# medvedevgroup/vargeno

Measured on AMD Instinct MI355X. Metric: reads/sec genotyped (whole node), hg38+dbSNP 30×; achieved HBM GB/s vs peak, higher is better.
Workload: dtype u64

## Files before the change

include/vargeno_hip.h:

```cpp
#ifndef VARGENO_HIP_H
#define VARGENO_HIP_H
#include <stddef.h>
#include <stdint.h>
#ifdef __cplusplus
extern "C" {
#endif

#define VG_OK        0
#define VG_EINVAL   -1
#define VG_EIO      -2
#define VG_ENOMEM   -3
#define VG_ENODEV   -4
#define VG_ETOOBIG  -5
#define VG_EBADREAD -6

typedef struct vg_index vg_index;

typedef struct {
	uint64_t n_ref;            const uint64_t *ref_kmer;  const uint32_t *ref_pos;  const uint8_t *ref_amb;
	uint64_t n_ref_aux;        const uint32_t *ref_aux;
	uint64_t n_snp;            const uint64_t *snp_kmer;  const uint32_t *snp_pos;
	const uint8_t *snp_info;   const uint8_t *snp_amb;    const uint8_t *snp_rf;    const uint8_t *snp_af;
	uint64_t n_snp_aux;        const uint32_t *snp_aux_pos;
	                           const uint8_t  *snp_aux_info;
// ... 122 lines not shown

int  vg_fastq_stream_begin_gzip(vg_index *ix);
int  vg_gzip_stream_stats(vg_index *ix, vg_gzip_stats *stats);
int  vg_fastq_stream_gzip_checkpoint(vg_index *ix, uint64_t text_offset, uint64_t *comp_bit_offset, uint64_t *ckpt_text_offset, uint8_t *window, uint32_t *window_len);

int  vg_fastq_submit(vg_index *ix, const uint8_t *text, uint64_t nbytes,
                     uint64_t *n_records, uint64_t *consumed, uint64_t *last_record_start);

typedef struct vg_packer vg_packer;
int  vg_packer_create(int host_threads, vg_packer **out);
void vg_packer_destroy(vg_packer *pk);
int  vg_packer_begin(vg_packer *pk);
uint64_t vg_packer_reads_cap(uint64_t nbytes);
uint64_t vg_packer_kmers_cap(uint64_t nbytes);
int  vg_packer_push(vg_packer *pk, const uint8_t *text, uint64_t nbytes, uint64_t *kmers, uint64_t kmers_cap, uint64_t *meta,
                    uint64_t *chunk_offsets, uint64_t reads_cap, uint64_t *n_reads, uint64_t *n_chunks, uint64_t *n_invalid);
int  vg_packer_end(vg_packer *pk, uint64_t *n_records, uint64_t *consumed, uint64_t *last_record_start, int *refused);

int  vg_sync(vg_index *ix);
int  vg_stats_get(vg_index *ix, vg_stats *out);
int  vg_set_stats(vg_index *ix, int enable);
int  vg_timing_get(vg_index *ix, vg_timing *out);
uint64_t vg_held_passes(const vg_index *ix);

uint64_t vg_num_sites(const vg_index *ix);
int  vg_sites_fetch(vg_index *ix, uint32_t *pos, uint8_t *ref_base, uint8_t *alt_base,
                    uint8_t *ref_freq, uint8_t *alt_freq);
int  vg_counts_fetch(vg_index *ix, uint8_t *ref_cnt, uint8_t *alt_cnt);
int  vg_counts_reset(vg_index *ix);

int  vg_sample_calls_fetch(vg_index *ix, uint8_t *gt, int32_t *gq, uint64_t *n_escaped);
int  vg_call_device(int device, const uint8_t *ref_cnt, const uint8_t *alt_cnt, const uint8_t *ref_freq, const uint8_t *alt_freq,
                    uint64_t n, double guard, uint8_t *gt, int32_t *gq, uint64_t *n_escaped);

typedef struct vg_gmatrix vg_gmatrix;
int  vg_gmatrix_create(int device, uint64_t n_sites, uint32_t n_samples, vg_gmatrix **out);
int  vg_gmatrix_set(vg_gmatrix *gm, uint32_t sample, const uint8_t *gt, const int32_t *gq, int32_t min_gq);
int  vg_gmatrix_pairs(vg_gmatrix *gm, uint64_t words_per_block, uint64_t *counts);
uint64_t vg_gmatrix_device_bytes(const vg_gmatrix *gm);
void vg_gmatrix_destroy(vg_gmatrix *gm);
int  vg_pairs_host(const uint8_t *gt, const int32_t *gq, uint64_t n_sites, uint32_t n_samples, int32_t min_gq, int threads, uint64_t *counts);

#ifndef VG_CPRIOR_ITERS
#define VG_CPRIOR_ITERS     8
#define VG_CPRIOR_PSEUDO    2.0
#define VG_CPRIOR_ITERS_MAX 64
// ... 80 lines not shown
```

vargeno_amd/_lib.py:

```python
from __future__ import annotations

import ctypes as C
import os

HERE = os.path.dirname(os.path.abspath(__file__))
LIB_PATH = os.environ.get("VARGENO_HIP_LIB") or os.path.join(HERE, "csrc", "libvargeno_hip.so")

VG_ERRORS = {-1: "VG_EINVAL", -2: "VG_EIO", -3: "VG_ENOMEM", -4: "VG_ENODEV", -5: "VG_ETOOBIG", -6: "VG_EBADREAD"}

STAT_FIELDS = ["reads", "reads_n", "reads_invalid", "passes", "passes_ok", "chunks", "gate_open",
               "refbf_pos", "snpbf_pos", "large_block", "ref_query", "snp_query", "ref_probe", "snp_probe",
               "scan_ref", "scan_snp", "scan_oob", "aux_ref", "aux_snp", "site_test", "ctx", "walks", "incr",
               "ingest_bytes", "overflow_reads", "overflow_deep", "alg_bytes"]

SYMBOLS = ["vg_last_error", "vg_build_id", "vg_device_count", "vg_device_memory", "vg_share_budget", "vg_link_rate", "vg_host_alloc_pinned", "vg_host_free_pinned", "vg_index_open", "vg_index_open_ex", "vg_index_plan", "vg_index_open_report", "vg_index_create", "vg_index_close",
           "vg_index_device_bytes", "vg_index_views", "vg_reads_submit", "vg_reads_process_device", "vg_reads_process_device_gated", "vg_reads_submit_packed", "vg_reads_submit_packed_async", "vg_read_store_create", "vg_read_store_push", "vg_read_store_flush", "vg_read_store_reads", "vg_read_store_bytes_used", "vg_reads_submit_store", "vg_read_store_destroy", "vg_fastq_submit", "vg_fastq_stream_begin", "vg_fastq_stream_begin_packed", "vg_fastq_stream_push", "vg_fastq_stream_end",
           "vg_packer_create", "vg_packer_destroy", "vg_packer_begin", "vg_packer_reads_cap", "vg_packer_kmers_cap", "vg_packer_push", "vg_packer_end", "vg_sync", "vg_stats_get",
           "vg_set_stats", "vg_timing_get", "vg_num_sites", "vg_sites_fetch", "vg_counts_fetch", "vg_counts_reset",
           "vg_counts_device_ptr", "vg_counts_allreduce", "vg_counts_allreduce_devices",
           "vg_samples_reserve", "vg_num_samples", "vg_sample_select", "vg_sample_selected", "vg_sample_reset", "vg_sample_invalid_reads",
           "vg_fastq_stream_begin_bgzf", "vg_fastq_stream_bgzf_locate", "vg_bgzf_inflate_device", "vg_bgzf_inflate_host", "vg_bgzf_scan_host",
           "vg_bgzf_deflate_bound", "vg_bgzf_deflate_host", "vg_bgzf_deflate_device",
           "vg_bgzf_deflate_host_coded", "vg_bgzf_deflate_device_coded", "vg_deflate_code_lengths_host", "vg_deflate_code_lengths_device",
           "vg_sample_calls_fetch", "vg_call_device",
           "vg_fastq_stream_begin_bam", "vg_bam_stream_stats", "vg_bam_frame_device", "vg_bam_to_fastq_host",
           "vg_gunzip_host", "vg_gunzip_device", "vg_gunzip_chunked_host", "vg_gunzip_pushed_host",
           "vg_fastq_stream_begin_gzip", "vg_gzip_stream_stats", "vg_fastq_stream_gzip_checkpoint",
           "vg_gmatrix_create", "vg_gmatrix_set", "vg_gmatrix_pairs", "vg_gmatrix_device_bytes", "vg_gmatrix_destroy", "vg_pairs_host",
           "vg_cprior_create", "vg_cprior_set", "vg_cprior_run", "vg_cprior_calls", "vg_cprior_device_bytes", "vg_cprior_destroy", "vg_cprior_host",
           "vg_jtext_create", "vg_jtext_destroy", "vg_jtext_device_bytes", "vg_jtext_set", "vg_jtext_text_bound", "vg_jtext_bgzf_bound", "vg_jtext_render", "vg_jtext_render_host",
           "vg_jtext_bgzf_begin", "vg_jtext_bgzf_text", "vg_jtext_bgzf_lines", "vg_jtext_bgzf_end",
           "vg_vcfidx_create", "vg_vcfidx_destroy", "vg_vcfidx_text_host", "vg_vcfidx_text_device", "vg_vcfidx_bgzf", "vg_vcfidx_bound", "vg_vcfidx_finish", "vg_vcfidx_error", "vg_vcfidx_stats",
           "vg_bgzf_deflate_device_indexed", "vg_jtext_bgzf_index",
           "vg_jtext_create_info", "vg_jtext_text_bound_info", "vg_jtext_render_host_info", "vg_jtext_counts", "vg_jtext_counts_host",
           "vg_held_passes"]

GZIP_STAT_FIELDS = ["members", "chunks", "guessed", "confirmed", "repaired", "tested", "slots_refused", "resume_bit"]


class VgStats(C.Structure):
    _fields_ = [(n, C.c_uint64) for n in STAT_FIELDS]

    def as_dict(self):
        return {n: int(getattr(self, n)) for n in STAT_FIELDS}


class VgGzipStats(C.Structure):
    _fields_ = [(n, C.c_uint64) for n in GZIP_STAT_FIELDS]

    def as_dict(self):
        return {n: int(getattr(self, n)) for n in GZIP_STAT_FIELDS}


class VgGzipOpts(C.Structure):
    _fields_ = [(n, C.c_uint64) for n in ("chunk_bytes", "slot_bytes", "max_ratio", "slot_max")]


class VgTiming(C.Structure):
# ... 183 lines not shown
        L.vg_vcfidx_text_host.argtypes = [vp, vp, C.c_uint64, C.c_int]
        L.vg_vcfidx_text_device.argtypes = [vp, C.c_int, vp, C.c_uint64]
        L.vg_vcfidx_bgzf.argtypes = [vp, vp, C.c_uint64]
        L.vg_vcfidx_bound.argtypes = [vp]
        L.vg_vcfidx_bound.restype = C.c_uint64
        L.vg_vcfidx_finish.argtypes = [vp, vp, C.c_uint64, C.POINTER(C.c_uint64)]
        L.vg_vcfidx_error.argtypes = [vp, C.POINTER(C.c_uint64)]
        L.vg_vcfidx_error.restype = C.c_char_p
        L.vg_vcfidx_stats.argtypes = [vp, vp]
        L.vg_bgzf_deflate_device_indexed.argtypes = [C.c_int, vp, C.c_uint64, C.c_uint32, C.c_int, C.c_int, vp, vp, C.c_uint64, C.POINTER(C.c_uint64)]
        L.vg_jtext_bgzf_index.argtypes = [vp, vp]
        L.vg_jtext_create_info.argtypes = [C.c_int, C.c_uint64, C.c_uint32, C.c_uint32, C.c_uint64, C.c_uint64, C.c_uint64, C.c_int, C.c_int, C.POINTER(vp)]
        L.vg_jtext_text_bound_info.argtypes = [C.c_uint64, C.c_uint64, C.c_uint32, C.c_int]
        L.vg_jtext_text_bound_info.restype = C.c_uint64
        L.vg_jtext_render_host_info.argtypes = [C.c_uint64, C.c_uint32, vp, vp, vp, C.c_uint64, vp, C.c_uint64, vp, C.c_uint64, C.c_int, C.c_int, vp, C.c_uint64, C.POINTER(C.c_uint64), C.POINTER(C.c_uint64)]
        L.vg_jtext_counts.argtypes = [vp, vp, C.c_uint64, vp, C.c_uint64, vp]
        L.vg_jtext_counts_host.argtypes = [C.c_uint64, C.c_uint32, vp, vp, vp, C.c_uint64, vp, C.c_uint64, vp]
        try:
            L.vg_held_passes.argtypes = [vp]
            L.vg_held_passes.restype = C.c_uint64
        except AttributeError:
            if not os.environ.get("VARGENO_HIP_LIB"):
                raise
        if not os.environ.get("VARGENO_HIP_LIB"):
            want = source_build_id()
            got = L.vg_build_id().decode()
            if want is not None and got != want:
                raise RuntimeError("stale %s: built from sources with id %s, the sources next to it have id %s -- rebuild with "
                                   "`python -c 'import __graft_entry__ as g; g.build()'`" % (LIB_PATH, got, want))
        _lib = L
    return _lib


LIB_SOURCES = [os.path.join(HERE, "..", "include", "vargeno_hip.h")] + [os.path.join(HERE, "csrc", f) for f in ("vg_device.h", "vg_wave.h", "vargeno_hip.hip", "vg_sort.hip", "vg_arena.h", "vg_hostpack.h", "vg_hostpack.cpp", "vg_allreduce_plan.h", "vg_hostpack_impl.h", "vg_hostpack_impl.inc", "vg_hostpack_avx2.cpp")]


def source_build_id():
    import hashlib

    h = hashlib.sha256()
    try:
        for f in LIB_SOURCES:
            with open(f, "rb") as fh:
                h.update(fh.read())
    except OSError:
        return None
# ... 7 lines not shown
```

vargeno_amd/api.py:

```python
from __future__ import annotations

import collections
import ctypes as C
import os
import re

import numpy as np

from . import _lib
from ._lib import VgIndexArrays, VgStats, VgTiming, check, lib


def _ptr(a):
    return a.ctypes.data_as(C.c_void_p)


class GenoIndex:

    def __init__(self, handle, device):
        self._h = handle
        self.device = device
        self._stores = []

    @classmethod
# ... 158 lines not shown
        self._stores = []

    def set_stats(self, enable):
        check(lib().vg_set_stats(self._h, 1 if enable else 0))

    def stats(self):
        s = VgStats()
        check(lib().vg_stats_get(self._h, C.byref(s)))
        return s.as_dict()

    def timing(self):
        t = VgTiming()
        check(lib().vg_timing_get(self._h, C.byref(t)))
        return dict(ms_total=float(t.ms_total), ms_pack=float(t.ms_pack), ms_main=float(t.ms_main), ms_tail=float(t.ms_tail), ms_deep_lists=float(t.ms_deep_lists), batches=int(t.batches))

    @property
    def held_passes(self):
        fn = getattr(lib(), "vg_held_passes", None)
        if fn is None:
            raise RuntimeError("the library named by VARGENO_HIP_LIB predates vg_held_passes")
        return int(fn(self._h))

    @property
    def num_sites(self):
        return int(lib().vg_num_sites(self._h))

    @property
    def device_bytes(self):
        return int(lib().vg_index_device_bytes(self._h))

    VIEW_NAMES = {1: "sec", 2: "mx", 4: "dx", 8: "snp_probe", 16: "snp_jg32", 32: "hx", 64: "snp_sig", 128: "sec_is_bf", 256: "ssec"}

    @property
    def views(self):
        m = int(lib().vg_index_views(self._h))
        return [n for b, n in sorted(self.VIEW_NAMES.items()) if m & b]

    def sites(self):
        n = self.num_sites
        pos = np.empty(n, np.uint32)
        u8 = [np.empty(n, np.uint8) for _ in range(4)]
        check(lib().vg_sites_fetch(self._h, _ptr(pos), *[_ptr(x) for x in u8]))
        return dict(pos=pos, ref_base=u8[0], alt_base=u8[1], ref_freq=u8[2], alt_freq=u8[3])

    def reserve_samples(self, n):
        check(lib().vg_samples_reserve(self._h, int(n)))
# ... 744 lines not shown
```

vargeno_amd/csrc/vargeno_hip.hip:

```cpp
#include "../../include/vargeno_hip.h"
#include "vg_device.h"
#include "vg_wave.h"
#include "vg_hostpack.h"
#include "vg_allreduce_plan.h"
#include "vg_arena.h"
#include "vg_inflate.h"
#include "vg_deflate.h"
#include "vg_bam.h"
#include "vg_gunzip.h"
#include "vg_caller.h"
#include "vg_pairs.h"
#include "vg_cprior.h"
#include "vg_jtext.h"
#include "vg_vcfidx.h"

#include <dlfcn.h>
#include <hip/hip_runtime.h>
#include <fcntl.h>
#include <stdio.h>
#include <stdlib.h>
#include <string.h>
#include <sys/stat.h>
#include <unistd.h>

// ... 1596 lines not shown
	LateStore late;
	uint32_t late_h[4] = {0, 0, 0, 0};
	bool late_dirty = false, late_stats = false;
	uint64_t late_reads_run = 0;
	bool spill_known = false;
	uint32_t spill_hint = 0;
	uint64_t cum[4] = {0, 0, 0, 0};
	uint8_t *d_clamped = nullptr;
	void *d_call_block = nullptr;
	const uint8_t *d_site_rf = nullptr, *d_site_af = nullptr;
	uint16_t *d_calls = nullptr;
	const vg_caller_tables *d_call_tab = nullptr;
	unsigned long long *d_call_esc = nullptr;
	unsigned long long *d_stats = nullptr;
	bool stats_enabled = true;
	bool force_generic = false;
	double t_pack = 0, t_main = 0, t_tail = 0, t_total = 0, t_w2 = 0; uint64_t t_batches = 0;
	int cus = 256;
	int lane_grid_blocks = 0, wave_grid = 0;
	uint32_t work_chunk = 128;
	uint32_t hold_pairs = VG_HOLD_PAIRS_DEFAULT;
	uint32_t wave_wgs = 0;
	uint64_t held_passes = 0;
	uint32_t w2_chunk = 8, w2_wpc = 3;
	bool w2_full_grid = false;
	FqStream *d_fq = nullptr;
	bool fq_open = false; int fq_prev_slot = -1;
	BgzfStream bz;
	bool fq_bgzf = false;
	struct GzipStream *gz = nullptr;
	bool fq_gzip = false;
	uint64_t max_device_bytes = 0;
	std::string plan_text;
	std::string aux_note;
	std::string open_report;
	vgp::Packer *packer = nullptr;
	bool fq_packed = false;
	uint64_t host_invalid = 0;
};

static thread_local vg_index *g_building = nullptr;
static thread_local double g_alloc_s = 0;

template <class T>
static int dev_alloc(vg_index *ix, T **p, uint64_t count, bool zero = false, bool plain = false)
{
// ... 1015 lines not shown
	if (!ix) return fail(VG_ENOMEM, "host allocation failed");
	ix->max_device_bytes = max_device_bytes;
	const double t0 = now_s();
	int rc = guarded([&] { return open_impl(prefix, device, ix); });
	if (rc) { vg_index_close(ix); return rc; }
	finish_construction(ix);
	char line[80];
	snprintf(line, sizeof line, "; vg_index_open %.2f s in all", now_s() - t0);
	ix->open_report += line;
	*out = ix;
	return VG_OK;
}

extern "C" const char *vg_index_plan(const vg_index *ix) { return ix ? ix->plan_text.c_str() : ""; }
extern "C" const char *vg_index_open_report(const vg_index *ix) { return ix ? ix->open_report.c_str() : ""; }

extern "C" int vg_index_open(const char *prefix, int device, vg_index **out)
{
	return vg_index_open_ex(prefix, device, env_budget(), out);
}
extern "C" uint64_t vg_index_device_bytes(const vg_index *ix) { return ix ? ix->dev_bytes : 0; }
extern "C" uint64_t vg_num_sites(const vg_index *ix) { return ix ? ix->n_sites : 0; }
extern "C" uint64_t vg_held_passes(const vg_index *ix) { return ix ? ix->held_passes : 0; }
extern "C" uint32_t vg_index_views(const vg_index *ix)
{
	if (!ix) return 0;
	const DevIndex &d = ix->d;
	return (d.sec3 ? VG_VIEW_SEC : 0u) | (d.sec_is_bf ? VG_VIEW_SEC_IS_BF : 0u) | (d.mx ? VG_VIEW_MX : 0u) | (d.dx ? VG_VIEW_DX : 0u) | (d.snp_probe ? VG_VIEW_SNP_PROBE : 0u) | (d.snp_jg32 ? VG_VIEW_SNP_JG32 : 0u) | (d.hx ? VG_VIEW_HX : 0u) | (d.snp_sig ? VG_VIEW_SNP_SIG : 0u) | (d.ssec3 ? VG_VIEW_SSEC : 0u);
}

template <class... A>
static void launch_lane(bool stats, unsigned grid, unsigned block, hipStream_t st, const A &...a)
{
	if (stats) vg_lane_kernel<true><<<grid, block, 0, st>>>(a...);
	else vg_lane_kernel<false><<<grid, block, 0, st>>>(a...);
}

static DevIndex plane_view(const vg_index *ix, uint32_t plane)
{
	DevIndex v = ix->d;
	v.cnt = ix->planes[plane].p.cnt; v.cnt4 = ix->planes[plane].p.cnt4;
	return v;
}

static int harvest(vg_index *ix, Slot &sl)
{
	if (!sl.busy) return VG_OK;
	HIP_TRY(hipEventSynchronize(sl.batch_done));
	const uint32_t resid = sl.lt_late ? sl.h_ctr.p[6] : sl.h_ctr.p[1];
	uint32_t *const r_list = sl.lt_late ? sl.listA.p : sl.listB.p, *const r_cnt = sl.lt_late ? &sl.ctr[6] : &sl.ctr[1];
	if (resid) ix->lane_tier_seen = true;
	if (resid && !sl.lt_enqueued) {
		launch_lane(sl.lt_stats, ix->big.s.nlanes / 64, 64, ix->tail2, plane_view(ix, sl.plane), ix->big.s, sl.lt_bases, sl.lt_quals, sl.lt_offsets, 0, r_list, r_cnt, sl.listC.p, &sl.ctr[2], ix->d_stats, nullptr, sl.lt_gate, sl.pk_kmer.p, sl.pk_meta.p, sl.lt_packed, nullptr, nullptr);
		HIP_TRY(hipGetLastError());
		HIP_TRY(hipMemcpyAsync(sl.h_ctr.p, sl.ctr, 32, hipMemcpyDeviceToHost, ix->tail2));
		HIP_TRY(hipStreamSynchronize(ix->tail2));
	}
	for (int i = 0; i < 4; i++) ix->cum[i] += sl.h_ctr.p[i];
	ix->held_passes += sl.h_ctr.p[CTR_HELD];
	ix->planes[sl.plane].invalid += sl.h_ctr.p[3];
	ix->spill_hint = std::max<uint32_t>(sl.h_ctr.p[0], ix->spill_hint / 2);
	ix->spill_known = true;
	float pack = 0, wave = 0, tail = 0, total = 0, w2 = 0;
	HIP_TRY(hipEventElapsedTime(&pack, sl.pack_begin, sl.pack_end)); HIP_TRY(hipEventElapsedTime(&wave, sl.wave_begin, sl.wave_end));
	HIP_TRY(hipEventElapsedTime(&tail, sl.wave_end, sl.batch_done)); HIP_TRY(hipEventElapsedTime(&total, sl.pack_begin, sl.batch_done)); HIP_TRY(hipEventElapsedTime(&w2, sl.wave_end, sl.deep_end));
	ix->t_pack += pack; ix->t_main += wave; ix->t_tail += tail; ix->t_total += total; ix->t_w2 += w2; ix->t_batches++;
	sl.busy = false;
	return VG_OK;
}

static int run_late_store(vg_index *ix)
{
	if (!ix->late_dirty || !ix->late.state) return VG_OK;
	unsigned long long st[2] = {0, 0};
	HIP_TRY(hipMemcpy(st, ix->late.state, 16, hipMemcpyDeviceToHost));
	ix->late_dirty = false;
	const uint64_t n = st[1];
	if (st[0] == 0) return VG_OK;
	if (n) {
		launch_lane(ix->late_stats, ix->big.s.nlanes / 64, 64, ix->tail, ix->d, ix->big.s, nullptr, nullptr, ix->late.offsets, n, nullptr, nullptr, ix->late.lost, ix->late.lost_n, ix->d_stats, nullptr, nullptr, ix->late.kmers, ix->late.meta, true, ix->d_planes, ix->late.tag);
		HIP_TRY(hipGetLastError());
	}
// ... 101 lines not shown
		if (sl.lt_late) {
			vg_late_collect<<<4, 256, 0, ix->tail>>>(ix->late, sl.pk_kmer.p, sl.pk_meta.p, d_offsets, sl.listB.p, &ctr[1], sl.listA.p, &ctr[6], sl.plane);
			ix->late_dirty = true; ix->late_stats = stats;
		}
	} else {
		sl.lt_late = false;
		const unsigned g1 = (unsigned)std::min<uint64_t>((n_reads + 255) / 256, (uint64_t)ix->lane_grid_blocks);
		if ((rc = begin_batch(sl, ix->stream, produced_on))) return rc;
		HIP_TRY(hipEventRecord(sl.pack_end, ix->stream));
		HIP_TRY(hipEventRecord(sl.wave_begin, ix->stream));
		launch_lane(stats, g1, 256, ix->stream, dv, ix->mid.s, d_bases, d_quals, d_offsets, n_reads, nullptr, d_n_reads, sl.listB.p, &ctr[1], ix->d_stats, packed ? nullptr : &ctr[3], d_gate, sl.pk_kmer.p, sl.pk_meta.p, packed, nullptr, nullptr);
		HIP_TRY(hipEventRecord(sl.wave_end, ix->stream));
		HIP_TRY(hipStreamWaitEvent(ix->tail, sl.wave_end, 0));
	}
	HIP_TRY(hipEventRecord(sl.deep_end, ix->tail));
	sl.lt_bases = d_bases; sl.lt_quals = d_quals; sl.lt_offsets = d_offsets; sl.lt_gate = d_gate; sl.lt_packed = packed; sl.lt_stats = stats;
	sl.lt_enqueued = ix->lane_tier_seen;
	hipStream_t lt = ix->tail;
	if (sl.lt_enqueued) {
		lt = ix->tail2;
		HIP_TRY(hipStreamWaitEvent(lt, sl.deep_end, 0));
		launch_lane(stats, ix->big.s.nlanes / 64, 64, lt, dv, ix->big.s, d_bases, d_quals, d_offsets, 0, sl.lt_late ? sl.listA.p : sl.listB.p, sl.lt_late ? &ctr[6] : &ctr[1], sl.listC.p, &ctr[2], ix->d_stats, nullptr, d_gate, sl.pk_kmer.p, sl.pk_meta.p, packed, nullptr, nullptr);
	}
	HIP_TRY(hipMemcpyAsync(sl.h_ctr.p, ctr, 32, hipMemcpyDeviceToHost, lt));
	HIP_TRY(hipEventRecord(sl.batch_done, lt));
	HIP_TRY(hipGetLastError());
	sl.busy = true;
	return VG_OK;
}

static int acquire_slot(vg_index *ix, Slot **out, uint32_t sample)
{
	Slot &sl = ix->slot[ix->next_slot];
	ix->next_slot = (ix->next_slot + 1) % NSLOT;
	int rc = harvest(ix, sl);
	if (rc) return rc;
	sl.plane = sample;
	*out = &sl;
	return VG_OK;
}

static int size_slot(Slot &sl, uint64_t n_reads, uint64_t n_chunks)
{
	int rc;
	if ((rc = sl.pk_kmer.reserve(n_chunks + 2, "packed reads"))) return rc;
	if ((rc = sl.pk_meta.reserve(n_reads + 1, "packed reads' flag words"))) return rc;
	return reserve_together({&sl.listA, &sl.listB, &sl.listC}, n_reads, "spill lists");
// ... 1669 lines not shown
		HIP_TRY(hipMemset(d_esc.p, 0, sizeof(unsigned long long)));
		vg_call_kernel<<<call_grid(n), VG_CALL_BLOCK>>>(d_cnt.p, d_rf.p, d_af.p, d_tab.p, n, guard, d_code.p, d_esc.p);
		HIP_TRY(hipGetLastError());
		HIP_TRY(hipDeviceSynchronize());
		unsigned long long esc = 0;
		HIP_TRY(hipMemcpy(code.data(), d_code.p, n * sizeof(uint16_t), hipMemcpyDeviceToHost));
		HIP_TRY(hipMemcpy(&esc, d_esc.p, sizeof esc, hipMemcpyDeviceToHost));
		resolve_calls(code.data(), ref_cnt, alt_cnt, ref_freq, alt_freq, n, gt, gq);
		if (n_escaped) *n_escaped = esc;
		return VG_OK;
	});
}

extern "C" int vg_counts_reset(vg_index *ix)
{
	if (!ix) return fail(VG_EINVAL, "null argument");
	{ int rc = finish_pending(ix); if (rc) return rc; }
	HIP_TRY(hipMemsetAsync(ix->d.cnt, 0, (2 * ix->n_sites + 2) * 4, ix->stream));
	for (size_t s = 1; s < ix->planes.size(); s++) HIP_TRY(hipMemsetAsync(ix->planes[s].p.cnt, 0, 2 * ix->n_sites * 4, ix->stream));
	for (Plane &pl : ix->planes) pl.invalid = 0;
	HIP_TRY(hipMemsetAsync(ix->d_stats, 0, S_COUNT * sizeof(unsigned long long), ix->stream));
	for (auto &c : ix->cum) c = 0;
	ix->held_passes = 0;
	ix->host_invalid = 0;
	HIP_TRY(hipStreamSynchronize(ix->stream));
	return VG_OK;
}

extern "C" int vg_counts_device_ptr(vg_index *ix, void **d_counts, uint64_t *n_u32)
{
	if (!ix || !d_counts || !n_u32) return fail(VG_EINVAL, "null argument");
	{ int rc = finish_pending(ix); if (rc) return rc; }
	*d_counts = sel_cnt(ix); *n_u32 = 2 * ix->n_sites;
	return VG_OK;
}

extern "C" uint32_t vg_num_samples(const vg_index *ix) { return ix ? (uint32_t)ix->planes.size() : 0; }
extern "C" uint32_t vg_sample_selected(const vg_index *ix) { return ix ? ix->cur_sample : 0; }
extern "C" int vg_sample_select(vg_index *ix, uint32_t sample)
{
	if (!ix) return fail(VG_EINVAL, "null argument");
	if (sample >= ix->planes.size()) return fail(VG_EINVAL, "sample %s is out of range: the handle has %s plane(s) (vg_samples_reserve)", std::to_string(sample).c_str(), std::to_string(ix->planes.size()).c_str());
	ix->cur_sample = sample;
	return VG_OK;
}
extern "C" int vg_samples_reserve(vg_index *ix, uint32_t n_samples)
// ... 1465 lines not shown
```

vargeno_amd/csrc/vg_wave.h:

```cpp
#pragma once
#include "vg_device.h"
#include "vg_acand.h"

#ifndef VG_WPE
#define VG_WPE 4
#endif
#ifndef VG_SCAN_W
#define VG_SCAN_W 2
#endif

#ifdef VG_STAGE_CLOCKS
#define VG_CLK(i) do { const long long t_ = clock64(); clk[i] += t_ - tlast; tlast = t_; } while (0)
#define VG_CLKW(i) do { __builtin_amdgcn_s_waitcnt(0); VG_CLK(i); } while (0)
#else
#define VG_CLK(i) do { } while (0)
#define VG_CLKW(i) do { } while (0)
#endif

#ifdef VG_STAGE_CLOCKS
__device__ unsigned long long vg_dbg_ovf[8];
#define VG_OVF(r) atomicAdd(&vg_dbg_ovf[(WPB > 1 ? 0 : 4) + (r)], 1ull)
#else
#define VG_OVF(r) do { } while (0)
#endif
// ... 4 lines not shown
#define VG_W1_ECAP 14
#endif
#ifndef VG_W1_NCAP
#define VG_W1_NCAP 6
#endif
#ifndef VG_W1_WPB
#define VG_W1_WPB 4
#endif
constexpr int W1_ECAP = VG_W1_ECAP, W1_NCAP = VG_W1_NCAP, W1_WPB = VG_W1_WPB;
constexpr int W3_ECAP = 48, W3_NCAP = 40;
constexpr uint32_t NOHIT = 0xFFFFFFFFu;
#ifndef VG_SEC_W
#define VG_SEC_W 8
#endif
constexpr int SEC_W = VG_SEC_W;
#ifndef VG_SEC_LONG
#define VG_SEC_LONG 256
#endif
constexpr uint32_t SEC_LONG = VG_SEC_LONG;
constexpr int PCAP = 32;
#ifndef VG_HOLD_PAIRS_DEFAULT
#define VG_HOLD_PAIRS_DEFAULT 12
#endif
constexpr int CTR_WORK_MAIN = 4, CTR_HELD = 7;
constexpr int HCAP = 4;

constexpr uint64_t PK_SKIP_N = 1ull << 62;
constexpr uint64_t PK_INVALID = 1ull << 63;
constexpr uint64_t PK_LONG = 1ull << 61;

__device__ inline uint32_t mk_meta(uint32_t chunk, uint32_t mod, bool neigh, uint32_t nbase) { return chunk | (mod << 5) | ((neigh ? 1u : 0u) << 10) | (nbase << 11); }

struct FuseIn {
	const uint8_t *bases, *quals;
	const uint32_t *gate;
	uint32_t *invalid_reads;
};
#ifndef VG_FUSE_PACK
#define VG_FUSE_PACK 0
#endif

template <bool WIDE> struct XKey { typedef uint32_t type; };
template <> struct XKey<true> { typedef uint64_t type; };
template <bool NARROW> struct KMask { typedef uint32_t type; };
template <> struct KMask<true> { typedef uint16_t type; };

template <bool STATS>
// ... 56 lines not shown
	uint32_t WORK_CHUNK = WORK_CHUNK_ARG;
	if constexpr (WPB == 1) if (read_ids) {
		const uint64_t fair = n_reads / (2ull * gridDim.x * WPB);
		if (fair > WORK_CHUNK) WORK_CHUNK = fair < 16 ? (uint32_t)fair : 16u;
	}
	const uint32_t POOL = WORK_CHUNK * (WPB > 1 ? WPB / 2 : 1);
	const uint32_t work_base = gridDim.x * POOL;
	if (threadIdx.x == 0) {
		const uint64_t p0 = (uint64_t)blockIdx.x * POOL, p1 = p0 + POOL < n_reads ? p0 + POOL : n_reads;
		Q_state = p0 < n_reads ? ((unsigned long long)p1 << 32) | p0 : 0ull;
		Q_lock = 0u; Q_done = 0u;
	}
	__syncthreads();
	uint32_t cursor = 0, end = 0;
	bool drained = false;

	bool active = false;
	constexpr bool HOLD = HOLDK && !STATS && !NOMX && WPB > 1;
	__shared__ uint8_t H_kcnt[HOLD ? 64 * WPB : 1];
	const uint32_t hold_pairs = HOLD ? (HOLD_PAIRS_ARG < (uint32_t)PCAP ? HOLD_PAIRS_ARG : (uint32_t)PCAP) : 0u;
	uint64_t heldm = 0ull;
	uint32_t held_passes = 0;
	const auto held_lane = [&heldm]() -> bool { return HOLD && __builtin_amdgcn_inverse_ballot_w64(heldm); };
#ifdef VG_STAGE_CLOCKS
	long long clk[12] = {0, 0, 0, 0, 0, 0, 0, 0, 0, 0, 0, 0}, tlast = clock64();
	uint32_t iters = 0, dbg_pairs = 0, dbg_items = 0, dbg_rounds = 0, dbg_dq = 0, dbg_rows = 0, dbg_large = 0, dbg_secbad = 0, dbg_holds = 0, dbg_flushes = 0;
#endif
	uint32_t rid = 0, n = 0, gates = 0, pass = 0;
	uint32_t slot0 = 0;
	LaneStats<STATS> tot, cur;
	tot.clear(); cur.clear();

	auto chunk_kmer = [&](uint32_t c) -> uint64_t {
		VG_VC_AS(VC_READS, pk_kmer + ((uint64_t)slot0 + (pass ? n - 1 - c : c)), 8);
		const uint64_t kf = pk_kmer[(uint64_t)slot0 + (pass ? n - 1 - c : c)];
		return pass ? revcomp64(kf) : kf;
	};

	auto chunk_kmer2 = [&](uint32_t c, uint64_t &k0, uint64_t &k1) {
		ulonglong2 v;
		VG_VC_AS(VC_READS, pk_kmer + ((uint64_t)slot0 + (pass ? n - 2 - c : c)), 16);
		__builtin_memcpy(&v, pk_kmer + ((uint64_t)slot0 + (pass ? n - 2 - c : c)), 16);
		k0 = pass ? revcomp64(v.y) : v.x;
		k1 = pass ? revcomp64(v.x) : v.y;
	};

// ... 62 lines not shown
							uint4 t[4];
							#pragma unroll
							for (uint32_t q = 0; q < 4; q++) if (q < 2 || two) t[q] = load_policy<false, uint4, 1>(src + 32 * c0 + 16 * q);
							#pragma unroll
							for (uint32_t z = 0; z < 2; z++) if (z == 0 || two) {
								const uint4 a = t[2 * z], b = t[2 * z + 1];
								const uint64_t k = (uint64_t)pack8(((uint64_t)a.y << 32) | a.x, bad) | ((uint64_t)pack8(((uint64_t)a.w << 32) | a.z, bad) << 16) |
								                   ((uint64_t)pack8(((uint64_t)b.y << 32) | b.x, bad) << 32) | ((uint64_t)pack8(((uint64_t)b.w << 32) | b.z, bad) << 48);
								dst[c0 + z] = k;
							}
						}
						if (fuse.gate) meta = n >= 32 ? fuse.gate[rid] : (fuse.gate[rid] & ((1u << n) - 1u));
						else for (uint32_t c0 = 0; c0 < n && c0 < 32; c0 += 4) {
							uint32_t q4;
							__builtin_memcpy(&q4, fuse.quals + off + c0, 4);
							for (uint32_t j = 0; j < 4 && c0 + j < n && c0 + j < 32; j++) if ((int)(int8_t)(q4 >> (8 * j)) - '8' < 0) meta |= 1ull << (c0 + j);
						}
						if (bad) meta |= classify_bad(src, n) == 1 ? PK_SKIP_N : PK_INVALID;
						if (n > 32) meta |= fuse.gate ? PK_INVALID : PK_LONG;
						if (meta & PK_INVALID) atomicAdd(fuse.invalid_reads, 1u);
						const_cast<uint64_t *>(pk_meta)[rid] = meta;
					} else meta = pk_meta[rid];
					gates = (uint32_t)meta;
					pass = 0;
					cur.clear();
					cur.add(S_READS, 1);
					cur.add(S_INGEST, 9 * n);
					if (meta & (PK_SKIP_N | PK_INVALID)) {
						cur.add((meta & PK_INVALID) ? S_READS_INVALID : S_READS_N, 1);
						if constexpr (STATS) for (int i = 0; i < S_COUNT; i++) tot.v[i] += cur.v[i];
					} else if ((meta & PK_LONG) || n > KMASK_CHUNKS) {
						overflow_list[atomicAdd(overflow_count, 1u)] = rid;
					} else {
						active = true;
					}
				}
			}
			cursor += take;
		}
		if (!__any(active)) { if (drained) break; continue; }
		VG_CLK(0);
#ifdef VG_STAGE_CLOCKS
		iters++;
#endif

		uint32_t kcnt = 0, ncnt = 0;
		uint32_t npend = 0;
		bool ovf = false;
		if (active && !held_lane()) {
			uint32_t hint = 0;
			auto key_find = [&](uint32_t q, uint32_t c, uint32_t lo, uint32_t hi, bool &dup, uint32_t qb = 0u) -> uint32_t {
				uint32_t e = (uint32_t)W_ECAP;
				const uint32_t cnt = hi - lo;
				if (cnt) {
					if (hint < lo || hint >= hi) hint = lo;
					for (uint32_t done = 0; done < cnt && e == (uint32_t)W_ECAP; done += 4) {
						uint32_t v[4], at[4];
						#pragma unroll
						for (uint32_t z = 0; z < 4; z++) { uint32_t i = hint + done + z; if (i >= hi) i -= cnt; if (i >= hi) i = lo; at[z] = i; v[z] = K_idx[i][col]; }
						#pragma unroll
						for (uint32_t z = 0; z < 4; z++) if (e == (uint32_t)W_ECAP && done + z < cnt && v[z] == q) e = at[z];
					}
				}
				if (e != (uint32_t)W_ECAP) {
					const uint32_t m = K_mask[e][col];
					if ((m >> c) & 1u) dup = true; else K_mask[e][col] = (kmask_t)(m | (1u << c) | qb);
					hint = e + 1u;
				}
				return e;
			};
			auto quiet_bit = [&](uint32_t hf, uint32_t c) -> uint32_t { return (hf & 6u) == 0u ? vg_quiet_chunks(hf, c, n) << KFREE : 0u; };
			auto push_exact = [&](uint32_t p, uint32_t c, uint32_t hf = 0u) {
// ... 91 lines not shown
						cur.add(S_CHUNKS, 1);
						emit_exact(c + z, rhit[z] != 0u, rpos[z], rhit[z] >> 1, shit[z] != 0u, spos[z], shit[z] >> 1);
					}
				}
			} else if (use_mx) {
				uint32_t k_strand = 0; bool k_pal = false;
				auto scan_bucket = [&](uint64_t k, uint32_t lo, uint32_t hi, uint4 first, bool &rhit, uint32_t &rpos, uint32_t &ramb, bool &shit, uint32_t &spos, uint32_t &samb) {
					const uint32_t key = (uint32_t)k;
					uint32_t ea = lo;
					if (hi - lo > 4) {
						uint32_t eb = hi;
						while (ea < eb) { const uint32_t m = ea + ((eb - ea) >> 1); if (d.mx[m].x < key) ea = m + 1; else eb = m; }
					}
					for (uint32_t e = ea; e < hi; e++) {
						const uint4 v = (e == lo) ? first : d.mx[e];
						if (v.x < key) continue;
						if (v.x > key) break;
						if (!(k_pal || ((v.z >> 3) & 1u) == k_strand)) continue;
						if (v.z & 1u) { shit = true; spos = v.y; samb = (v.z >> 1) & 1u; }
						else { rhit = true; rpos = v.y; ramb = (v.z >> 1) & 1u; }
					}
				};
				if (d.dx) {
					constexpr uint32_t RC_BAD = 0xFFFFu;
					uint32_t rc_top = pass != 0u ? RC_BAD : (uint32_t)W_ECAP;
					for (uint32_t c = 0; c < n; c += 4) {
						const uint32_t m = n - c < 4u ? n - c : 4u;
						uint64_t kq[4] = {0, 0, 0, 0};
						if (m >= 2) chunk_kmer2(c, kq[0], kq[1]); else kq[0] = chunk_kmer(c);
						if (m >= 4) chunk_kmer2(c + 2, kq[2], kq[3]); else if (m == 3) kq[2] = chunk_kmer(c + 2);
						uint32_t sbits = 0;
						#pragma unroll
						for (uint32_t z = 0; z < 4; z++) {
							const uint64_t kk = kq[z], rr = revcomp64(kk), ck = kk < rr ? kk : rr;
							sbits |= (kk != ck ? 1u : 0u) << z | (kk == rr ? 1u : 0u) << (4u + z);
							kq[z] = fmix64(ck);
						}
						VG_CLKW(9);
						using xkey_t = typename XKey<SDX>::type;
						const uint32_t dxb = SDX ? d.dx_bits : 32u;
						auto ekey = [](const uint4 &e) -> xkey_t { if constexpr (SDX) return ((uint64_t)(e.z & 0xFFFF0000u) << 32) | e.x; else return e.x; };
						auto ecnt = [](const uint4 &b) -> uint32_t { return SDX ? (b.z >> 8) & 0xFFu : b.z >> 8; };
						uint4 bq[4];
						xkey_t kx[4];
						#pragma unroll
						for (uint32_t z = 0; z < 4; z++) {
							bq[z] = make_uint4(0, 0, 0, 0);
// ... 160 lines not shown
										bool dup = false;
										if (key_find(q, cc, rev ? rc_top : 0u, rev ? (uint32_t)W_ECAP : kcnt, dup, qb) == (uint32_t)W_ECAP) {
											if (rev ? rc_top > kcnt : kcnt < (uint32_t)W_ECAP) {
												const uint32_t at = rev ? rc_top - 1u : kcnt;
												K_idx[at][col] = q; K_mask[at][col] = (kmask_t)((1u << cc) | qb);
												if (rev) rc_top = at; else { kcnt++; hint = kcnt; }
											} else if (rev) rc_top = RC_BAD;
											else { VG_OVF(0); ovf = true; }
										} else if (dup) { if (rev) rc_top = RC_BAD; else { VG_OVF(2); ovf = true; } }
									}
								}
							}
							if (!rc_ok) rc_top = RC_BAD;
							if (z0 == 0u) { bq[0] = bq[2]; bq[1] = bq[3]; kx[0] = kx[2]; kx[1] = kx[3]; more[0] = more[2]; more[1] = more[3]; }
						}
#endif
					}
					if (pass == 0u && kcnt == 0u && rc_top != RC_BAD && !ovf) {
						const uint32_t nrc = (uint32_t)W_ECAP - rc_top;
						for (uint32_t i = 0; i < nrc; i++) { K_idx[i][col] = K_idx[rc_top + i][col]; K_mask[i][col] = K_mask[rc_top + i][col]; }
						kcnt = nrc;
						pass = 1u;
					}
				} else
				for (uint32_t c = 0; c < n; c += 2) {
					const bool two = c + 1 < n;
					uint64_t k0 = chunk_kmer(c), k1 = two ? chunk_kmer(c + 1) : 0;
					uint32_t st0, st1; bool pl0, pl1;
					{ const uint64_t r = revcomp64(k0), ck = k0 < r ? k0 : r; st0 = k0 != ck; pl0 = k0 == r; k0 = fmix64(ck); }
					{ const uint64_t r = revcomp64(k1), ck = k1 < r ? k1 : r; st1 = k1 != ck; pl1 = k1 == r; k1 = fmix64(ck); }
					uint32_t lo0, hi0, lo1 = 0, hi1 = 0;
					jg_pair(d.mx_jg, k0 >> 32, lo0, hi0);
					if (two) jg_pair(d.mx_jg, k1 >> 32, lo1, hi1);
					uint4 f0 = make_uint4(0, 0, 0, 0), f1 = f0;
					if (lo0 < hi0) f0 = d.mx[lo0];
					if (lo1 < hi1) f1 = d.mx[lo1];
					uint32_t rpos = 0, ramb = 0, spos = 0, samb = 0;
					bool rhit = false, shit = false;
					cur.add(S_CHUNKS, 1);
					k_strand = st0; k_pal = pl0;
					scan_bucket(k0, lo0, hi0, f0, rhit, rpos, ramb, shit, spos, samb);
					emit_exact(c, rhit, rpos, ramb, shit, spos, samb);
					if (two) {
						rhit = shit = false;
						cur.add(S_CHUNKS, 1);
						k_strand = st1; k_pal = pl1;
// ... 731 lines not shown
							ni++;
							c = mt & 31u; mod = (mt >> 5) & 31u;
							if (wp - 32u * c != target) continue;
						}
						cur.add(S_WALKS, 1);
						if ((uint64_t)wp + 32 > d.pile_len) continue;
						const uint64_t kk = chunk_kmer(c);
						uint4 pw[2];
						load_pile_window(d, wp, pw);
						walk_matches(pw, kk, wp, mod, count);
					}
					}
					}
				}
			}
			if (ovf) {
				overflow_list[atomicAdd(overflow_count, 1u)] = rid;
				active = false;
			} else if (processed || pass == 1) {
				if constexpr (STATS) for (int i = 0; i < S_COUNT; i++) tot.v[i] += cur.v[i];
				active = false;
			} else {
				pass = 1;
			}
		}
		VG_WAVE_SYNC();
		VG_CLK(5);
	}
#ifdef VG_STAGE_CLOCKS
	{ const uint32_t dq = wave_sum<false>(dbg_dq); if (!STATS && lane == 0 && (blockIdx.x % 97u) == 0 && wv == 0) printf("DBG blk %u iters %u pairs %u items %u rounds %u dualq %u large %u secbad %u holds %u flushes %u\n", blockIdx.x, iters, dbg_pairs, dbg_items, dbg_rounds, dq, dbg_large, dbg_secbad, dbg_holds, dbg_flushes); }
	if (!STATS && lane == 0 && (blockIdx.x % 97u) == 0 && wv == 0)
		printf("CLK blk %u iters %u refill %lld A %lld B0 %lld B1 %lld vote %lld walk %lld wload %lld wloop %lld watom %lld Akmer %lld Adx %lld Ascan %lld ecap %d\n", blockIdx.x, iters, clk[0], clk[1], clk[2], clk[3], clk[4], clk[5], clk[6], clk[7], clk[8], clk[9], clk[10], clk[11], W_ECAP);
#endif
	if constexpr (STATS) {
		for (int i = 0; i < S_COUNT; i++) if (tot.v[i]) atomicAdd(&stats[i], (unsigned long long)tot.v[i]);
	}
	if constexpr (HOLD) if (held_passes && lane == 0) atomicAdd(work_next + (CTR_HELD - CTR_WORK_MAIN), held_passes);
}

#undef lane
#undef col

template <bool STATS, int W_ECAP, int W_NCAP, int WPB, bool SDX = false>
__global__ __launch_bounds__(64 * WPB) __attribute__((amdgpu_waves_per_eu(WPB > 1 ? VG_WPE : 1))) void vg_wave_kernel(DevIndex d, const uint64_t *__restrict__ pk_kmer, const uint64_t *__restrict__ pk_meta,
                                                     const uint64_t *__restrict__ offsets, uint64_t n_reads_arg,
                                                     const uint32_t *__restrict__ read_ids, const uint32_t *__restrict__ n_ids,
                                                     uint32_t *overflow_list, uint32_t *overflow_count, uint32_t *work_next, const uint32_t WORK_CHUNK_ARG, const uint32_t HOLD_PAIRS_ARG, unsigned long long *stats, const FuseIn fuse)
{
	vg_wave_body<STATS, W_ECAP, W_NCAP, WPB, false, SDX, true>(d, pk_kmer, pk_meta, offsets, n_reads_arg, read_ids, n_ids, overflow_list, overflow_count, work_next, WORK_CHUNK_ARG, HOLD_PAIRS_ARG, stats, fuse);
}

template <int W_ECAP, int W_NCAP, int WPB, bool SDX>
__global__ __launch_bounds__(64 * WPB) __attribute__((amdgpu_waves_per_eu(WPB > 1 ? VG_WPE : 1))) void vg_wave_kernel_plain(DevIndex d, const uint64_t *__restrict__ pk_kmer, const uint64_t *__restrict__ pk_meta,
                                                     const uint64_t *__restrict__ offsets, uint64_t n_reads_arg,
                                                     const uint32_t *__restrict__ read_ids, const uint32_t *__restrict__ n_ids,
                                                     uint32_t *overflow_list, uint32_t *overflow_count, uint32_t *work_next, const uint32_t WORK_CHUNK_ARG, const uint32_t HOLD_PAIRS_ARG, unsigned long long *stats, const FuseIn fuse)
{
	vg_wave_body<false, W_ECAP, W_NCAP, WPB, false, SDX, false>(d, pk_kmer, pk_meta, offsets, n_reads_arg, read_ids, n_ids, overflow_list, overflow_count, work_next, WORK_CHUNK_ARG, HOLD_PAIRS_ARG, stats, fuse);
}

template <int W_ECAP, int W_NCAP, int WPB>
__global__ __launch_bounds__(64 * WPB) __attribute__((amdgpu_waves_per_eu(WPB > 1 ? VG_WPE : 1))) void vg_wave_kernel_big(DevIndex d, const uint64_t *__restrict__ pk_kmer, const uint64_t *__restrict__ pk_meta,
// ... 9 lines not shown
```

Baseline: 4.006 billion.

## Carry first-pass RC candidate list into retry pass to skip re-lookup

When a read needs a second pass, the kernel now stores the first pass's reverse-complement candidate boundary in the upper 16 bits of the gates word. On retry it compacts the K_idx/K_mask entries and skips the whole lookup stage for that pass. A carried-pass counter is added to the device counters, copied back in a larger counter readback, and exposed through the C and Python APIs. This trades extra register/state bookkeeping and a wider counter copy for avoiding repeated index probing on retried reads.

```diff
diff --git a/include/vargeno_hip.h b/include/vargeno_hip.h
--- a/include/vargeno_hip.h
+++ b/include/vargeno_hip.h
@@ -168,6 +168,7 @@
 int  vg_set_stats(vg_index *ix, int enable);
 int  vg_timing_get(vg_index *ix, vg_timing *out);
 uint64_t vg_held_passes(const vg_index *ix);
+uint64_t vg_carried_passes(const vg_index *ix);
 
 uint64_t vg_num_sites(const vg_index *ix);
 int  vg_sites_fetch(vg_index *ix, uint32_t *pos, uint8_t *ref_base, uint8_t *alt_base,
diff --git a/vargeno_amd/_lib.py b/vargeno_amd/_lib.py
--- a/vargeno_amd/_lib.py
+++ b/vargeno_amd/_lib.py
@@ -33,7 +33,7 @@
            "vg_vcfidx_create", "vg_vcfidx_destroy", "vg_vcfidx_text_host", "vg_vcfidx_text_device", "vg_vcfidx_bgzf", "vg_vcfidx_bound", "vg_vcfidx_finish", "vg_vcfidx_error", "vg_vcfidx_stats",
            "vg_bgzf_deflate_device_indexed", "vg_jtext_bgzf_index",
            "vg_jtext_create_info", "vg_jtext_text_bound_info", "vg_jtext_render_host_info", "vg_jtext_counts", "vg_jtext_counts_host",
-           "vg_held_passes"]
+           "vg_held_passes", "vg_carried_passes"]
 
 GZIP_STAT_FIELDS = ["members", "chunks", "guessed", "confirmed", "repaired", "tested", "slots_refused", "resume_bit"]
 
@@ -263,6 +263,12 @@
         except AttributeError:
             if not os.environ.get("VARGENO_HIP_LIB"):
                 raise
+        try:
+            L.vg_carried_passes.argtypes = [vp]
+            L.vg_carried_passes.restype = C.c_uint64
+        except AttributeError:
+            if not os.environ.get("VARGENO_HIP_LIB"):
+                raise
         if not os.environ.get("VARGENO_HIP_LIB"):
             want = source_build_id()
             got = L.vg_build_id().decode()
diff --git a/vargeno_amd/api.py b/vargeno_amd/api.py
--- a/vargeno_amd/api.py
+++ b/vargeno_amd/api.py
@@ -204,6 +204,13 @@
         return int(fn(self._h))
 
     @property
+    def carried_passes(self):
+        fn = getattr(lib(), "vg_carried_passes", None)
+        if fn is None:
+            raise RuntimeError("the library named by VARGENO_HIP_LIB predates vg_carried_passes")
+        return int(fn(self._h))
+
+    @property
     def num_sites(self):
         return int(lib().vg_num_sites(self._h))
 
diff --git a/vargeno_amd/csrc/vargeno_hip.hip b/vargeno_amd/csrc/vargeno_hip.hip
--- a/vargeno_amd/csrc/vargeno_hip.hip
+++ b/vargeno_amd/csrc/vargeno_hip.hip
@@ -1642,6 +1642,7 @@
 	uint32_t hold_pairs = VG_HOLD_PAIRS_DEFAULT;
 	uint32_t wave_wgs = 0;
 	uint64_t held_passes = 0;
+	uint64_t carried_passes = 0;
 	uint32_t w2_chunk = 8, w2_wpc = 3;
 	bool w2_full_grid = false;
 	FqStream *d_fq = nullptr;
@@ -2703,6 +2704,7 @@
 extern "C" uint64_t vg_index_device_bytes(const vg_index *ix) { return ix ? ix->dev_bytes : 0; }
 extern "C" uint64_t vg_num_sites(const vg_index *ix) { return ix ? ix->n_sites : 0; }
 extern "C" uint64_t vg_held_passes(const vg_index *ix) { return ix ? ix->held_passes : 0; }
+extern "C" uint64_t vg_carried_passes(const vg_index *ix) { return ix ? ix->carried_passes : 0; }
 extern "C" uint32_t vg_index_views(const vg_index *ix)
 {
 	if (!ix) return 0;
@@ -2734,11 +2736,15 @@
 	if (resid && !sl.lt_enqueued) {
 		launch_lane(sl.lt_stats, ix->big.s.nlanes / 64, 64, ix->tail2, plane_view(ix, sl.plane), ix->big.s, sl.lt_bases, sl.lt_quals, sl.lt_offsets, 0, r_list, r_cnt, sl.listC.p, &sl.ctr[2], ix->d_stats, nullptr, sl.lt_gate, sl.pk_kmer.p, sl.pk_meta.p, sl.lt_packed, nullptr, nullptr);
 		HIP_TRY(hipGetLastError());
-		HIP_TRY(hipMemcpyAsync(sl.h_ctr.p, sl.ctr, 32, hipMemcpyDeviceToHost, ix->tail2));
+		HIP_TRY(hipMemcpyAsync(sl.h_ctr.p, sl.ctr, 4 * CTR_COPIED, hipMemcpyDeviceToHost, ix->tail2));
 		HIP_TRY(hipStreamSynchronize(ix->tail2));
 	}
 	for (int i = 0; i < 4; i++) ix->cum[i] += sl.h_ctr.p[i];
 	ix->held_passes += sl.h_ctr.p[CTR_HELD];
+	ix->carried_passes += sl.h_ctr.p[CTR_CARRIED];
+#ifdef VG_RETRY_CENSUS
+	fprintf(stderr, "RETRY_CENSUS carried %u retries %u usable %u usable_empty %u\n", sl.h_ctr.p[CTR_CARRIED], sl.h_ctr.p[CTR_CARRIED + 1], sl.h_ctr.p[CTR_CARRIED + 2], sl.h_ctr.p[CTR_CARRIED + 3]);
+#endif
 	ix->planes[sl.plane].invalid += sl.h_ctr.p[3];
 	ix->spill_hint = std::max<uint32_t>(sl.h_ctr.p[0], ix->spill_hint / 2);
 	ix->spill_known = true;
@@ -2886,7 +2892,7 @@
 		HIP_TRY(hipStreamWaitEvent(lt, sl.deep_end, 0));
 		launch_lane(stats, ix->big.s.nlanes / 64, 64, lt, dv, ix->big.s, d_bases, d_quals, d_offsets, 0, sl.lt_late ? sl.listA.p : sl.listB.p, sl.lt_late ? &ctr[6] : &ctr[1], sl.listC.p, &ctr[2], ix->d_stats, nullptr, d_gate, sl.pk_kmer.p, sl.pk_meta.p, packed, nullptr, nullptr);
 	}
-	HIP_TRY(hipMemcpyAsync(sl.h_ctr.p, ctr, 32, hipMemcpyDeviceToHost, lt));
+	HIP_TRY(hipMemcpyAsync(sl.h_ctr.p, ctr, 4 * CTR_COPIED, hipMemcpyDeviceToHost, lt));
 	HIP_TRY(hipEventRecord(sl.batch_done, lt));
 	HIP_TRY(hipGetLastError());
 	sl.busy = true;
@@ -4602,6 +4608,7 @@
 	HIP_TRY(hipMemsetAsync(ix->d_stats, 0, S_COUNT * sizeof(unsigned long long), ix->stream));
 	for (auto &c : ix->cum) c = 0;
 	ix->held_passes = 0;
+	ix->carried_passes = 0;
 	ix->host_invalid = 0;
 	HIP_TRY(hipStreamSynchronize(ix->stream));
 	return VG_OK;
diff --git a/vargeno_amd/csrc/vg_wave.h b/vargeno_amd/csrc/vg_wave.h
--- a/vargeno_amd/csrc/vg_wave.h
+++ b/vargeno_amd/csrc/vg_wave.h
@@ -50,7 +50,8 @@
 #ifndef VG_HOLD_PAIRS_DEFAULT
 #define VG_HOLD_PAIRS_DEFAULT 12
 #endif
-constexpr int CTR_WORK_MAIN = 4, CTR_HELD = 7;
+constexpr int CTR_WORK_MAIN = 4, CTR_WORK_DEEP = 5, CTR_HELD = 7, CTR_CARRIED = 8;
+constexpr int CTR_COPIED = 12;
 constexpr int HCAP = 4;
 
 constexpr uint64_t PK_SKIP_N = 1ull << 62;
@@ -153,6 +154,17 @@
 	uint64_t heldm = 0ull;
 	uint32_t held_passes = 0;
 	const auto held_lane = [&heldm]() -> bool { return HOLD && __builtin_amdgcn_inverse_ballot_w64(heldm); };
+#ifdef VG_NO_RETRY_CARRY
+	constexpr bool CARRY = false;
+#else
+	constexpr bool CARRY = !STATS && !NOMX;
+#endif
+	constexpr uint32_t RC_BAD = 0xFFFFu;
+#define RC_ROOM (WPB > 1 || n <= 16u)
+	uint32_t carried_passes = 0;
+#ifdef VG_RETRY_CENSUS
+	uint32_t cen_retry = 0, cen_usable = 0, cen_empty = 0;
+#endif
 #ifdef VG_STAGE_CLOCKS
 	long long clk[12] = {0, 0, 0, 0, 0, 0, 0, 0, 0, 0, 0, 0}, tlast = clock64();
 	uint32_t iters = 0, dbg_pairs = 0, dbg_items = 0, dbg_rounds = 0, dbg_dq = 0, dbg_rows = 0, dbg_large = 0, dbg_secbad = 0, dbg_holds = 0, dbg_flushes = 0;
@@ -261,6 +273,7 @@
 						const_cast<uint64_t *>(pk_meta)[rid] = meta;
 					} else meta = pk_meta[rid];
 					gates = (uint32_t)meta;
+					if constexpr (CARRY) if (RC_ROOM) gates |= RC_BAD << 16;
 					pass = 0;
 					cur.clear();
 					cur.add(S_READS, 1);
@@ -286,7 +299,13 @@
 		uint32_t kcnt = 0, ncnt = 0;
 		uint32_t npend = 0;
 		bool ovf = false;
-		if (active && !held_lane()) {
+		bool carried = false;
+		if constexpr (CARRY) {
+			carried = active && pass != 0u && RC_ROOM && (gates >> 16) != RC_BAD;
+			if (carried) { kcnt = gates >> 16; gates |= RC_BAD << 16; }
+			carried_passes += (uint32_t)__popcll(__ballot(carried));
+		}
+		if (active && !held_lane() && !carried) {
 			uint32_t hint = 0;
 			auto key_find = [&](uint32_t q, uint32_t c, uint32_t lo, uint32_t hi, bool &dup, uint32_t qb = 0u) -> uint32_t {
 				uint32_t e = (uint32_t)W_ECAP;
@@ -424,7 +443,6 @@
 					}
 				};
 				if (d.dx) {
-					constexpr uint32_t RC_BAD = 0xFFFFu;
 					uint32_t rc_top = pass != 0u ? RC_BAD : (uint32_t)W_ECAP;
 					for (uint32_t c = 0; c < n; c += 4) {
 						const uint32_t m = n - c < 4u ? n - c : 4u;
@@ -631,6 +649,7 @@
 						kcnt = nrc;
 						pass = 1u;
 					}
+					if constexpr (CARRY) if (RC_ROOM) gates = (gates & 0xFFFFu) | ((pass == 0u && !ovf && rc_top != RC_BAD && rc_top >= kcnt ? rc_top : RC_BAD) << 16);
 				} else
 				for (uint32_t c = 0; c < n; c += 2) {
 					const bool two = c + 1 < n;
@@ -1408,6 +1427,19 @@
 				active = false;
 			} else {
 				pass = 1;
+				if constexpr (CARRY) {
+					const uint32_t rct = gates >> 16;
+					const bool usable = RC_ROOM && rct != RC_BAD;
+#ifdef VG_RETRY_CENSUS
+					cen_retry++; cen_usable += usable ? 1u : 0u; cen_empty += usable && rct == (uint32_t)W_ECAP ? 1u : 0u;
+#endif
+					if (usable) {
+						const uint32_t nrc = (uint32_t)W_ECAP - rct;
+						for (uint32_t i = 0; i < nrc; i++) { K_idx[i][col] = K_idx[rct + i][col]; K_mask[i][col] = K_mask[rct + i][col]; }
+						if (nrc == 0u) active = false;
+						else gates = (gates & 0xFFFFu) | (nrc << 16);
+					}
+				}
 			}
 		}
 		VG_WAVE_SYNC();
@@ -1422,8 +1454,17 @@
 		for (int i = 0; i < S_COUNT; i++) if (tot.v[i]) atomicAdd(&stats[i], (unsigned long long)tot.v[i]);
 	}
 	if constexpr (HOLD) if (held_passes && lane == 0) atomicAdd(work_next + (CTR_HELD - CTR_WORK_MAIN), held_passes);
+	if constexpr (CARRY) {
+		uint32_t *const blk = work_next - (WPB > 1 ? CTR_WORK_MAIN : CTR_WORK_DEEP);
+		if (carried_passes && lane == 0) atomicAdd(blk + CTR_CARRIED, carried_passes);
+#ifdef VG_RETRY_CENSUS
+		cen_retry = wave_sum<false>(cen_retry); cen_usable = wave_sum<false>(cen_usable); cen_empty = wave_sum<false>(cen_empty);
+		if (cen_retry && lane == 0) { atomicAdd(blk + CTR_CARRIED + 1, cen_retry); atomicAdd(blk + CTR_CARRIED + 2, cen_usable); atomicAdd(blk + CTR_CARRIED + 3, cen_empty); }
+#endif
+	}
 }
 
+#undef RC_ROOM
 #undef lane
 #undef col
 
```

Result: slower. 3.952 billion (-1.4%).
